# graz-dev/llms-on-kubernetes

Hardware: AMD Instinct MI355X
Metric: output tok/s through gateway (p50 TTFT reported) (higher is better)
Workload: dtype bf16

## Files before the change

csrc/kernels/prefill_gemm_packed.hip:

```cpp
#include "hipserve/common.h"
#include "hipserve/kernels.h"

namespace hipserve {

constexpr int PW_T = 256;

constexpr int PW_GM = 8;
HS_DEVICE void pw_tile(int L, int tiles_m, int tiles_n, int& tm, int& tn) {
  const int grp = L / (PW_GM * tiles_n), first = grp * PW_GM;
  const int gsz = min(PW_GM, tiles_m - first);
  const int r = L - first * tiles_n;
  tm = first + r % gsz;
  tn = r / gsz;
}

HS_DEVICE void pw_barrier() {
  asm volatile("s_waitcnt lgkmcnt(0)" ::: "memory");
  __builtin_amdgcn_s_barrier();
  asm volatile("" ::: "memory");
}

HS_DEVICE void pw_mfma(f32x4& acc, const u32x4& w, const u32x4& x) {
  asm volatile("v_mfma_f32_16x16x32_bf16 %0, %1, %2, %0" : "+a"(acc) : "v"(w), "v"(x));
}

struct PwTile {
  __amdgpu_buffer_rsrc_t w, x;
  int m0, t;
  int xo[8];
};

template <int WM, bool kGroup, bool kGather = false>
HS_DEVICE PwTile pw_make(int L, int tiles_m, int tiles_n, int wn, const unsigned short* X, long ldx,
                         const unsigned short* Wp, int M, int ntiles, int KS, const PwGroup& grp) {
  constexpr int WN = 4 / WM, BM = 128 * WM;
  int tm, tn;
  pw_tile(L, tiles_m, tiles_n, tm, tn);
  PwTile T;
  T.m0 = tm * BM;
  T.t = tn * WN + wn;
  const int tl = min(T.t, ntiles - 1);
  if constexpr (kGroup) Wp += (long)__builtin_amdgcn_readfirstlane(grp.tile_expert[tm]) * grp.estride;
  T.w = __builtin_amdgcn_make_buffer_rsrc((void*)(Wp + (long)tl * KS * 32768), 0, KS * 65536, 0x00020000);
  if constexpr (kGather) {
    const int bytes = (int)((long)grp.x_rows * ldx * 2);
    T.x = __builtin_amdgcn_make_buffer_rsrc((void*)X, 0, bytes, 0x00020000);
    const int tid = threadIdx.x;
#pragma unroll
    for (int p = 0; p < BM / 32; ++p) {
      const int row = T.m0 + p * 32 + (tid >> 3);
      const int s = row < M ? grp.gather_slots[row] : -1;
      T.xo[p] = (s >= 0 ? (s / grp.gather_k) * (int)ldx * 2 : bytes) + (tid & 7) * 16;
    }
  } else {
    T.x = __builtin_amdgcn_make_buffer_rsrc((void*)(X + (long)T.m0 * ldx), 0,
                                            (int)((long)min(BM, M - T.m0) * ldx * 2), 0x00020000);
  }
  return T;
}

template <int WM, int EPI, bool kGroup, int RW, bool LDLY = false, bool kGather = false>
__global__ __launch_bounds__(PW_T) __attribute__((amdgpu_waves_per_eu(1, 1))) void pgw_kernel(
    const unsigned short* __restrict__ X, long ldx, const unsigned short* __restrict__ Wp,
    unsigned short* __restrict__ C, long ldc, int M, int N, int K, int tiles_m, int tiles_n,
    const unsigned short* __restrict__ bias, PwGroup grp) {
  constexpr int WN = 4 / WM, BM = 128 * WM, STAGE = BM * 128, XP = BM / 32;
  __shared__ __attribute__((aligned(1024))) unsigned char lds[2 * STAGE];
  const int tid = threadIdx.x, lane = tid & 63;
  const int wave = __builtin_amdgcn_readfirstlane(tid >> 6);
  const int wm = wave / WN, wn = wave - (wave / WN) * WN;
  const int ntiles = (N + 127) >> 7;
  const int KS = K >> 8, nq = K >> 5, nst = K >> 6;
  if constexpr (kGroup) tiles_m = min(tiles_m, __builtin_amdgcn_readfirstlane(*grp.num_tiles));
  const int total = tiles_m * tiles_n, G = gridDim.x;
  const int r = xcd_remap(blockIdx.x, G);
  if (r >= total) return;

  PwTile cur = pw_make<WM, kGroup, kGather>(r, tiles_m, tiles_n, wn, X, ldx, Wp, M, ntiles, KS, grp);
  PwTile nxt = r + G < total ? pw_make<WM, kGroup, kGather>(r + G, tiles_m, tiles_n, wn, X, ldx, Wp, M, ntiles, KS, grp) : cur;

  const int wvo = lane * 16;
  auto wload = [&](int q, int rg) -> u32x4 {
    const bool n = q >= nq;
    q = n ? q - nq : q;
    return __builtin_amdgcn_raw_buffer_load_b128(n ? nxt.w : cur.w, wvo, (q >> 3) * 65536 + rg * 8192 + (q & 7) * 1024,
                                                 0);
  };
  int xvo[XP];
#pragma unroll
  for (int p = 0; p < XP; ++p) xvo[p] = (p * 32 + (tid >> 3)) * (int)ldx * 2 + (tid & 7) * 16;
  const int xdo = (tid >> 3) * 128 + (((tid & 7) ^ ((tid >> 4) & 7)) * 16);
  constexpr int XS = RW / 2;
  u32x4 xst[XS][XP];
  auto xload = [&](int st, u32x4 (&xs)[XP]) {
    const bool n = st >= nst;
    st = n ? st - nst : st;
#pragma unroll
    for (int p = 0; p < XP; ++p)
      xs[p] = __builtin_amdgcn_raw_buffer_load_b128(n ? nxt.x : cur.x, kGather ? (n ? nxt.xo[p] : cur.xo[p]) : xvo[p],
                                                    st * 128, 0);
  };
  auto xstore = [&](int buf, const u32x4 (&xs)[XP]) {
#pragma unroll
    for (int p = 0; p < XP; ++p) *reinterpret_cast<u32x4*>(lds + buf * STAGE + p * 4096 + xdo) = xs[p];
  };
  const int fr = lane & 15, fq = lane >> 4, sw = (fr >> 1) & 7;
  const int foff = (wm * 128 + fr) * 128;
  const int ch[2] = {(fq ^ sw) * 16, ((4 + fq) ^ sw) * 16};
  auto xfrag = [&](int buf, int h, int i) -> u32x4 {
    return *reinterpret_cast<const u32x4*>(lds + buf * STAGE + foff + i * 2048 + ch[h]);
  };

  f32x4 acc[8][8];
  u32x4 w[RW][8], xa[8], xb[8];
  int wvoj[RW];
#pragma unroll
  for (int j = 0; j < RW; ++j) wvoj[j] = wvo + j * 1024;

  xload(0, xst[0]);
  xstore(0, xst[0]);
#pragma unroll
  for (int s = 1; s <= XS; ++s) xload(s, xst[s % XS]);
#pragma unroll
  for (int j = 0; j < RW; ++j)
#pragma unroll
    for (int rg = 0; rg < 8; ++rg) w[j][rg] = wload(j, rg);
  pw_barrier();
#pragma unroll
  for (int i = 0; i < 8; ++i) xa[i] = xfrag(0, 0, i);

  auto slot = [&](auto jc, int s0, const __amdgpu_buffer_rsrc_t& wrs, int wk) {
    constexpr int J = decltype(jc)::value, H = J & 1;
    const int s = s0 + J / 2, buf = s & 1;
    constexpr int XI = (J / 2 + 1) % XS;
#pragma unroll
    for (int rg = 0; rg < 8; ++rg) {
#pragma unroll
      for (int i = 0; i < 8; ++i) pw_mfma(acc[rg][i], w[J][rg], H ? xb[i] : xa[i]);
      if constexpr (LDLY) {
        if (rg > 0) w[J][rg - 1] = __builtin_amdgcn_raw_buffer_load_b128(wrs, wvoj[J], wk + (rg - 1) * 8192, 0);
        if (rg == 7) w[J][7] = __builtin_amdgcn_raw_buffer_load_b128(wrs, wvoj[J], wk + 7 * 8192, 0);
      } else {
        w[J][rg] = __builtin_amdgcn_raw_buffer_load_b128(wrs, wvoj[J], wk + rg * 8192, 0);
      }
      if constexpr (H == 0) {
        xb[rg] = xfrag(buf, 1, rg);
        if (rg == 2) xstore(buf ^ 1, xst[XI]);
        if (rg == 3) xload(s + 1 + XS, xst[XI]);
      } else {
        xa[rg] = xfrag(buf ^ 1, 0, rg);
      }
      __builtin_amdgcn_sched_barrier(0);
    }
    if constexpr (H == 0) pw_barrier();
  };
  using I0 = std::integral_constant<int, 0>;
  using I1 = std::integral_constant<int, 1>;
  using I2 = std::integral_constant<int, 2>;
  using I3 = std::integral_constant<int, 3>;

  for (int L = r;;) {
#pragma unroll
    for (int rg = 0; rg < 8; ++rg)
#pragma unroll
      for (int i = 0; i < 8; ++i) acc[rg][i] = f32x4{0.f, 0.f, 0.f, 0.f};
    for (int q0 = 0; q0 < nq; q0 += RW) {
      const int s0 = q0 >> 1;
      const bool wn = q0 + RW >= nq;
      const int wq = wn ? q0 + RW - nq : q0 + RW;
      const __amdgpu_buffer_rsrc_t wrs = wn ? nxt.w : cur.w;
      const int wk = (wq >> 3) * 65536 + (wq & 7) * 1024;
      slot(I0(), s0, wrs, wk);
      slot(I1(), s0, wrs, wk);
      if constexpr (RW == 4) {
        slot(I2(), s0, wrs, wk);
        slot(I3(), s0, wrs, wk);
      }
    }

    asm volatile("s_nop 7\n\ts_nop 7\n\ts_nop 7\n\ts_nop 7" ::: "memory");
    const int t = cur.t, mb = cur.m0 + wm * 128 + fr;
    if (t < ntiles) {
      if constexpr (EPI == PW_EPI_GLU || EPI == PW_EPI_GEGLU) {
        const int I = N >> 1;
#pragma unroll
        for (int i = 0; i < 8; ++i) {
          const int m = mb + 16 * i;
          if (m >= M) continue;
#pragma unroll
          for (int rg = 0; rg < 4; ++rg) {
            const int c = t * 64 + rg * 16 + 4 * fq;
            unsigned short o[4];
#pragma unroll
            for (int j = 0; j < 4; ++j) {
              const unsigned short g = f32_to_bf16(acc[rg][i][j]), u = f32_to_bf16(acc[rg + 4][i][j]);
              o[j] = EPI == PW_EPI_GEGLU ? gelu_mul1(g, u) : silu_mul1(g, u);
            }
            if (c < I)
              *reinterpret_cast<uint2*>(C + (long)m * ldc + c) =
                  uint2{(unsigned)o[0] | ((unsigned)o[1] << 16), (unsigned)o[2] | ((unsigned)o[3] << 16)};
          }
        }
      } else {
#pragma unroll
        for (int rg = 0; rg < 8; ++rg) {
          const int n = t * 128 + rg * 16 + 4 * fq;
          if (n >= N) continue;
          float bv[4] = {0.f, 0.f, 0.f, 0.f};
          if (bias != nullptr)
#pragma unroll
            for (int j = 0; j < 4; ++j) bv[j] = n + j < N ? bf16_to_f32(bias[n + j]) : 0.f;
#pragma unroll
          for (int i = 0; i < 8; ++i) {
            const int m = mb + 16 * i;
            if (m >= M) continue;
            uint2* dst = reinterpret_cast<uint2*>(C + (long)m * ldc + n);
            float o[4];
            if constexpr (EPI == PW_EPI_ADD) {
              const uint2 rv = *dst;
              const unsigned short rr[4] = {(unsigned short)(rv.x & 0xffff), (unsigned short)(rv.x >> 16),
                                            (unsigned short)(rv.y & 0xffff), (unsigned short)(rv.y >> 16)};
#pragma unroll
              for (int j = 0; j < 4; ++j) o[j] = bf16_to_f32(f32_to_bf16(acc[rg][i][j])) + bf16_to_f32(rr[j]);
            } else {
#pragma unroll
              for (int j = 0; j < 4; ++j) o[j] = acc[rg][i][j] + bv[j];
            }
            *dst = uint2{pack_bf16x2(o[0], o[1]), pack_bf16x2(o[2], o[3])};
          }
        }
      }
    }
    L += G;
    if (L >= total) break;
    cur = nxt;
    if (L + G < total) nxt = pw_make<WM, kGroup, kGather>(L + G, tiles_m, tiles_n, wn, X, ldx, Wp, M, ntiles, KS, grp);
  }
}

bool launch_prefill_gemm_packed(int epi, void* C, long ldc, const void* X, long ldx, const void* Wp, int M, int N,
                                int K, const void* bias, int wm, int grid_req, hipStream_t s, const PwGroup* group,
                                int rw) {
  const PwGroup grp = group != nullptr ? *group : PwGroup{nullptr, nullptr, 0};
  const bool grouped = group != nullptr;
  const bool gather = grouped && grp.gather_slots != nullptr;
  if (grouped && (bias != nullptr || epi == PW_EPI_ADD)) return false;
  if (gather && (grp.gather_k < 1 || (long)grp.x_rows * ldx * 2 >= (1L << 31) - 4096)) return false;
  if (M < 1 || N < 1 || K < 256 || K % 256 || (wm != 1 && wm != 2) || (rw != 2 && rw != 4 && rw != 5)) return false;
  const bool glu = epi == PW_EPI_GLU || epi == PW_EPI_GEGLU;
  if (glu && (N % 128 || bias != nullptr)) return false;
  if (epi == PW_EPI_ADD && bias != nullptr) return false;
  if ((long)(K / 256) * 65536 >= (1L << 31) || (long)128 * wm * ldx * 2 >= (1L << 31)) return false;
  const int BM = 128 * wm, WN = 4 / wm;
  const int tiles_m = (M + BM - 1) / BM, tiles_n = ((N + 127) / 128 + WN - 1) / WN;
  static int ncu = 0;
  if (ncu == 0) {
    int dev = 0;
    (void)hipGetDevice(&dev);
    if (hipDeviceGetAttribute(&ncu, hipDeviceAttributeMultiprocessorCount, dev) != hipSuccess || ncu < 1) ncu = 256;
  }
  const int total = tiles_m * tiles_n;
  const dim3 grid(min(total, grid_req > 0 ? grid_req : ncu));
  auto* x = static_cast<const unsigned short*>(X);
  auto* w = static_cast<const unsigned short*>(Wp);
  auto* c = static_cast<unsigned short*>(C);
  auto* b = static_cast<const unsigned short*>(bias);
#define PW_LAUNCH1(WM_, E_, RW_)                                                                               \
  do {                                                                                                         \
    if (gather)                                                                                                \
      pgw_kernel<WM_, E_, true, 4, false, true><<<grid, PW_T, 0, s>>>(x, ldx, w, c, ldc, M, N, K, tiles_m, tiles_n, b, grp); \
    else if (grouped)                                                                                          \
      pgw_kernel<WM_, E_, true, RW_><<<grid, PW_T, 0, s>>>(x, ldx, w, c, ldc, M, N, K, tiles_m, tiles_n, b, grp);  \
    else                                                                                                       \
      pgw_kernel<WM_, E_, false, RW_><<<grid, PW_T, 0, s>>>(x, ldx, w, c, ldc, M, N, K, tiles_m, tiles_n, b, grp); \
  } while (0)
#define PW_LAUNCH(WM_, E_)                                                                                   \
  do {                                                                                                       \
    if (rw == 4)                                                                                             \
      PW_LAUNCH1(WM_, E_, 4);                                                                                \
    else if (rw == 2)                                                                                        \
      PW_LAUNCH1(WM_, E_, 2);                                                                                \
    else if (grouped)                                                                                        \
      pgw_kernel<WM_, E_, true, 4, true><<<grid, PW_T, 0, s>>>(x, ldx, w, c, ldc, M, N, K, tiles_m, tiles_n, b, grp);  \
    else                                                                                                     \
      pgw_kernel<WM_, E_, false, 4, true><<<grid, PW_T, 0, s>>>(x, ldx, w, c, ldc, M, N, K, tiles_m, tiles_n, b, grp); \
  } while (0)
#define PW_EPIS(WM_)                                          \
  switch (epi) {                                              \
    case PW_EPI_STORE: PW_LAUNCH(WM_, PW_EPI_STORE); return true; \
    case PW_EPI_ADD: PW_LAUNCH(WM_, PW_EPI_ADD); return true;     \
    case PW_EPI_GLU: PW_LAUNCH(WM_, PW_EPI_GLU); return true;     \
    case PW_EPI_GEGLU: PW_LAUNCH(WM_, PW_EPI_GEGLU); return true; \
    default: return false;                                    \
  }
  if (wm == 1) {
    PW_EPIS(1)
  }
  PW_EPIS(2)
#undef PW_EPIS
#undef PW_LAUNCH
#undef PW_LAUNCH1
}

}
```

csrc/torch_bindings.cpp:

```cpp
#include <torch/library.h>
#include <ATen/ATen.h>
#include <ATen/hip/impl/HIPGuardImplMasqueradingAsCUDA.h>
#include <ATen/hip/impl/HIPStreamMasqueradingAsCUDA.h>

#include "hipserve/kernels.h"

namespace {

hipStream_t cur_stream() {
  return c10::hip::getCurrentHIPStreamMasqueradingAsCUDA().stream();
}

#define CHECK_DEV(x) TORCH_CHECK((x).is_cuda(), #x " must be a GPU tensor")
#define CHECK_BF16(x) TORCH_CHECK((x).scalar_type() == at::kBFloat16, #x " must be bf16")
#define CHECK_ROWMAJOR(x) TORCH_CHECK((x).stride(-1) == 1, #x " must have unit inner stride")
#define CHECK_CONTIG(x) TORCH_CHECK((x).is_contiguous(), #x " must be contiguous")

static void e4m3_out_args(const c10::optional<at::Tensor>& out8, const c10::optional<at::Tensor>& xs8,
                          const at::Tensor& out, void** o8, float** x8, const char* who);

void rmsnorm(at::Tensor& out, const at::Tensor& x, const at::Tensor& weight, double eps,
             const c10::optional<at::Tensor>& out8, const c10::optional<at::Tensor>& xs8) {
  CHECK_DEV(x); CHECK_BF16(x); CHECK_BF16(out); CHECK_ROWMAJOR(x); CHECK_ROWMAJOR(out);
  TORCH_CHECK(x.dim() == 2 && out.dim() == 2, "rmsnorm expects 2-D [rows, hidden]");
// ... 612 lines not shown
  TORCH_CHECK(logits.dim() == 2 && (logits.scalar_type() == at::kBFloat16 || logits.scalar_type() == at::kFloat));
  const int rows = logits.size(0);
  TORCH_CHECK(nreq.scalar_type() == at::kInt && nreq.numel() >= rows);
  TORCH_CHECK(out_ids.scalar_type() == at::kInt && out_lp.scalar_type() == at::kFloat && out_ids.dim() == 2 &&
              out_ids.sizes() == out_lp.sizes() && out_ids.size(0) >= rows && out_ids.is_contiguous() &&
              out_lp.is_contiguous() && out_ids.size(1) <= 64);
  c10::hip::HIPGuardMasqueradingAsCUDA g(logits.device());
  hipserve::launch_top_logprobs(logits.data_ptr(), logits.scalar_type() == at::kBFloat16, logits.stride(0), rows,
                                logits.size(1), nreq.data_ptr<int>(), out_ids.data_ptr<int>(),
                                out_lp.data_ptr<float>(), out_ids.size(1), cur_stream());
}

bool car_error(int64_t state) { return hipserve::car_error(reinterpret_cast<void*>(state)); }

void car_destroy(int64_t state) { hipserve::car_destroy(reinterpret_cast<void*>(state)); }

void fill_uniform(at::Tensor& out, int64_t row0, int64_t col0, int64_t gcols, int64_t key, double scale) {
  CHECK_DEV(out); CHECK_BF16(out);
  TORCH_CHECK(out.dim() == 2 && out.stride(1) == 1, "fill_uniform: 2-D row-major view");
  c10::hip::HIPGuardMasqueradingAsCUDA g(out.device());
  hipserve::launch_fill_uniform(out.data_ptr(), out.stride(0), out.size(0), out.size(1), row0, col0, gcols,
                                (unsigned int)(key & 0xffffffffu), (float)scale, cur_stream());
}

void stage_copy(const std::vector<at::Tensor>& dst, const std::vector<at::Tensor>& src, int64_t device) {
  TORCH_CHECK(dst.size() == src.size() && dst.size() <= (size_t)hipserve::kMaxStageCopies,
              "stage_copy: matching lists of at most 8 tensors");
  hipserve::StageCopyArgs a{};
  a.n = (int)dst.size();
  auto addr = [](const at::Tensor& t, bool& host) -> void* {
    TORCH_CHECK(t.is_contiguous(), "stage_copy: tensors must be contiguous");
    if (t.is_cuda()) { host = false; return t.data_ptr(); }
    TORCH_CHECK(t.is_pinned(), "stage_copy: host tensors must be pinned");
    host = true;
    void* d = nullptr;
    TORCH_CHECK(hipHostGetDevicePointer(&d, t.data_ptr(), 0) == hipSuccess && d,
                "stage_copy: pinned tensor has no device mapping");
    return d;
  };
  for (int i = 0; i < a.n; ++i) {
    const size_t nb = dst[i].nbytes();
    TORCH_CHECK(nb == src[i].nbytes() && nb % 4 == 0, "stage_copy: pair ", i, " byte sizes differ or not 4-aligned");
    bool hd = false, hs = false;
    a.dst[i] = addr(dst[i], hd);
    a.src[i] = addr(src[i], hs);
    a.words[i] = (long)(nb / 4);
    a.host_mask |= (hs ? 1u : 0u) << (2 * i);
    a.host_mask |= (hd ? 1u : 0u) << (2 * i + 1);
  }
  c10::hip::HIPGuardMasqueradingAsCUDA g((c10::DeviceIndex)device);
  hipserve::launch_stage_copy(a, cur_stream());
}

void decode_gemm(at::Tensor& out, const at::Tensor& x, const at::Tensor& w, at::Tensor& ws, int64_t rt,
                 int64_t splits) {
  CHECK_DEV(x); CHECK_BF16(x); CHECK_BF16(w); CHECK_BF16(out); CHECK_ROWMAJOR(x); CHECK_ROWMAJOR(out);
  CHECK_CONTIG(w);
  const int M = x.size(0), K = x.size(1), N = w.size(0);
  TORCH_CHECK(w.size(1) == K && out.size(0) == M && out.size(1) == N, "decode_gemm: shape mismatch");
  TORCH_CHECK(M >= 1 && M <= 64, "decode_gemm: 1 <= M <= 64");
  TORCH_CHECK(splits >= 1 && K % (256 * splits) == 0, "decode_gemm: K must be a multiple of 256*splits");
  TORCH_CHECK(N % 4 == 0 && out.stride(0) % 4 == 0 && x.stride(0) % 8 == 0, "decode_gemm: alignment");
  if (splits > 1) {
    TORCH_CHECK(ws.scalar_type() == at::kFloat && ws.is_contiguous() && ws.numel() >= splits * M * N && N % 8 == 0,
                "decode_gemm: fp32 workspace of S*M*N (N % 8 == 0) required for split-K");
  }
  c10::hip::HIPGuardMasqueradingAsCUDA g(x.device());
  TORCH_CHECK(hipserve::launch_decode_gemm(out.data_ptr(), out.stride(0),
                                           splits > 1 ? ws.data_ptr<float>() : nullptr, x.data_ptr(), x.stride(0),
                                           w.data_ptr(), M, N, K, rt, splits, false, 0, cur_stream()),
              "decode_gemm: unsupported (rt, K/splits): rt in {1,2}, K/splits = 256*{1,2,4,7,8,12,16,21}");
}

void decode_gemm_packed(at::Tensor& out, const at::Tensor& x, const at::Tensor& wp, at::Tensor& ws, int64_t N,
                        int64_t rt, int64_t splits) {
  CHECK_DEV(x); CHECK_BF16(x); CHECK_BF16(wp); CHECK_BF16(out); CHECK_ROWMAJOR(x); CHECK_ROWMAJOR(out);
  CHECK_CONTIG(wp);
  const int M = x.size(0), K = x.size(1);
  TORCH_CHECK(K % 256 == 0 && wp.numel() == (N + 127) / 128 * 128 * K, "decode_gemm_packed: packed size mismatch");
  TORCH_CHECK(out.size(0) == M && out.size(1) == N, "decode_gemm_packed: out shape");
  TORCH_CHECK(M >= 1 && M <= 64, "decode_gemm_packed: 1 <= M <= 64");
  TORCH_CHECK(splits >= 1 && K % (256 * splits) == 0, "decode_gemm_packed: K must be a multiple of 256*splits");
  TORCH_CHECK(N % 4 == 0 && out.stride(0) % 4 == 0 && x.stride(0) % 8 == 0, "decode_gemm_packed: alignment");
  if (splits > 1) {
    TORCH_CHECK(ws.scalar_type() == at::kFloat && ws.is_contiguous() && ws.numel() >= splits * M * N && N % 8 == 0,
                "decode_gemm_packed: fp32 workspace of S*M*N (N % 8 == 0) required for split-K");
  }
  c10::hip::HIPGuardMasqueradingAsCUDA g(x.device());
  TORCH_CHECK(hipserve::launch_decode_gemm(out.data_ptr(), out.stride(0),
                                           splits > 1 ? ws.data_ptr<float>() : nullptr, x.data_ptr(), x.stride(0),
                                           wp.data_ptr(), M, N, K, rt, splits, true, 0, cur_stream()),
              "decode_gemm_packed: unsupported (rt, K/splits)");
}

void decode_gemm_partial(at::Tensor& ws, const at::Tensor& x, const at::Tensor& w, int64_t N, int64_t rt,
                         int64_t splits, bool packed) {
  CHECK_DEV(x); CHECK_BF16(x); CHECK_BF16(w); CHECK_ROWMAJOR(x); CHECK_CONTIG(w);
  const int M = x.size(0), K = x.size(1);
  if (packed) {
    TORCH_CHECK(w.numel() == (N + 127) / 128 * 128 * K, "decode_gemm_partial: packed size mismatch");
  } else {
    TORCH_CHECK(w.dim() == 2 && w.size(0) == N && w.size(1) == K, "decode_gemm_partial: w [N, K]");
  }
  TORCH_CHECK(M >= 1 && M <= 64 && K % (256 * splits) == 0 && N % 8 == 0 && x.stride(0) % 8 == 0,
              "decode_gemm_partial: shape / alignment");
  TORCH_CHECK(ws.scalar_type() == at::kFloat && ws.is_contiguous() && ws.numel() >= splits * M * N,
              "decode_gemm_partial: ws must hold S*M*N fp32");
  c10::hip::HIPGuardMasqueradingAsCUDA g(x.device());
  TORCH_CHECK(hipserve::launch_decode_gemm(nullptr, N, ws.data_ptr<float>(), x.data_ptr(), x.stride(0), w.data_ptr(),
                                           M, N, K, rt, splits, packed, hipserve::DG_PARTIAL, cur_stream()),
              "decode_gemm_partial: unsupported (rt, K/splits)");
}

void decode_gemm_glu(at::Tensor& act, const at::Tensor& x, const at::Tensor& wp, at::Tensor& ws, int64_t N,
                     int64_t rt, int64_t splits) {
  CHECK_DEV(x); CHECK_BF16(x); CHECK_BF16(wp); CHECK_BF16(act); CHECK_ROWMAJOR(x); CHECK_ROWMAJOR(act);
  CHECK_CONTIG(wp);
  const int M = x.size(0), K = x.size(1);
  TORCH_CHECK(N % 128 == 0 && wp.numel() == N * K && K % (256 * splits) == 0, "decode_gemm_glu: shapes");
  TORCH_CHECK(act.size(0) == M && act.size(1) == N / 2 && act.stride(0) % 8 == 0, "decode_gemm_glu: act [M, N/2]");
  TORCH_CHECK(M >= 1 && M <= 64 && x.stride(0) % 8 == 0, "decode_gemm_glu: 1 <= M <= 64");
  if (splits > 1) {
    TORCH_CHECK(ws.scalar_type() == at::kFloat && ws.is_contiguous() && ws.numel() >= splits * M * N,
                "decode_gemm_glu: ws must hold S*M*N fp32");
  }
  c10::hip::HIPGuardMasqueradingAsCUDA g(x.device());
  TORCH_CHECK(hipserve::launch_decode_gemm(act.data_ptr(), act.stride(0), splits > 1 ? ws.data_ptr<float>() : nullptr,
                                           x.data_ptr(), x.stride(0), wp.data_ptr(), M, N, K, rt, splits, true,
                                           hipserve::DG_GLU, cur_stream()),
              "decode_gemm_glu: unsupported (rt, K/splits)");
}



void prefill_gemm_packed(at::Tensor& out, const at::Tensor& x, const at::Tensor& wp, int64_t N, int64_t epi,
                         const c10::optional<at::Tensor>& bias, int64_t wm, int64_t grid, int64_t rw) {
  CHECK_DEV(x); CHECK_BF16(x); CHECK_BF16(wp); CHECK_BF16(out); CHECK_ROWMAJOR(x); CHECK_ROWMAJOR(out);
  TORCH_CHECK(wp.is_contiguous(), "prefill_gemm_packed: packed weight must be contiguous");
  const int M = x.size(0), K = x.size(1);
  TORCH_CHECK(K % 256 == 0 && wp.numel() == (N + 127) / 128 * 128 * K, "prefill_gemm_packed: wp = pack(w[N, K % 256])");
  TORCH_CHECK(x.stride(0) % 8 == 0 && out.stride(0) % 4 == 0, "prefill_gemm_packed: alignment");
  const bool glu = epi == 2 || epi == 3;
  TORCH_CHECK(out.size(0) == M && out.size(1) == (glu ? N / 2 : N), "prefill_gemm_packed: out shape");
  const void* bp = nullptr;
  if (bias.has_value()) {
    CHECK_BF16((*bias));
    TORCH_CHECK(bias->numel() == N && bias->is_contiguous(), "prefill_gemm_packed: bias [N]");
    bp = bias->data_ptr();
  }
  c10::hip::HIPGuardMasqueradingAsCUDA g(x.device());
  TORCH_CHECK(hipserve::launch_prefill_gemm_packed((int)epi, out.data_ptr(), out.stride(0), x.data_ptr(), x.stride(0),
                                                   wp.data_ptr(), M, (int)N, K, bp, (int)wm, (int)grid, cur_stream(),
                                                   nullptr, (int)rw),
              "prefill_gemm_packed: unsupported (glu needs N % 128, bias only with epi 0, 32-bit offsets)");
}

void prefill_gemm_packed_grouped(at::Tensor& out, const at::Tensor& x, const at::Tensor& wp, int64_t N, int64_t epi,
                                 const at::Tensor& tile_expert, const at::Tensor& num_tiles, int64_t wm, int64_t rw,
                                 const c10::optional<at::Tensor>& gather_slots, int64_t gather_k) {
  CHECK_DEV(x); CHECK_BF16(x); CHECK_BF16(wp); CHECK_BF16(out); CHECK_ROWMAJOR(x); CHECK_ROWMAJOR(out);
  TORCH_CHECK(wp.dim() == 2 && wp.is_contiguous(), "prefill_gemm_packed_grouped: wp [E, packed]");
  const bool gather = gather_slots.has_value() && gather_slots->numel() > 0;
  if (gather)
    TORCH_CHECK(gather_slots->scalar_type() == at::kInt && gather_slots->is_contiguous() &&
                    gather_slots->numel() == out.size(0) && gather_k >= 1 && x.stride(0) % 8 == 0,
                "prefill_gemm_packed_grouped: gather_slots [slot rows] int32, gather_k >= 1");
  const int M = gather ? out.size(0) : x.size(0), K = x.size(1);
  TORCH_CHECK(K % 256 == 0 && wp.size(1) == (N + 127) / 128 * 128 * K, "prefill_gemm_packed_grouped: wp per expert");
  TORCH_CHECK(M % (128 * wm) == 0 && tile_expert.numel() >= M / (128 * wm), "prefill_gemm_packed_grouped: tiles");
  TORCH_CHECK(tile_expert.scalar_type() == at::kInt && num_tiles.scalar_type() == at::kInt, "int32 tile tables");
  const bool glu = epi == 2 || epi == 3;
  TORCH_CHECK(epi == 0 || glu, "prefill_gemm_packed_grouped: store or glu epilogue");
  TORCH_CHECK(out.size(0) == M && out.size(1) == (glu ? N / 2 : N), "prefill_gemm_packed_grouped: out shape");
  c10::hip::HIPGuardMasqueradingAsCUDA g(x.device());
  hipserve::PwGroup grp{tile_expert.data_ptr<int>(), num_tiles.data_ptr<int>(), (long)wp.size(1)};
  if (gather) {
    grp.gather_slots = gather_slots->data_ptr<int>();
    grp.gather_k = (int)gather_k;
    grp.x_rows = (int)x.size(0);
  }
  TORCH_CHECK(hipserve::launch_prefill_gemm_packed((int)epi, out.data_ptr(), out.stride(0), x.data_ptr(), x.stride(0),
                                                   wp.data_ptr(), M, (int)N, K, nullptr, (int)wm, 0, cur_stream(),
                                                   &grp, (int)rw),
              "prefill_gemm_packed_grouped: unsupported");
}

void prefill_gemm_f8(at::Tensor& out, const at::Tensor& xq, const at::Tensor& xs, const std::vector<at::Tensor>& q,
                     const std::vector<at::Tensor>& rs, int64_t epi) {
  CHECK_DEV(xq); CHECK_CONTIG(xq); CHECK_CONTIG(xs); CHECK_BF16(out); CHECK_ROWMAJOR(out);
  TORCH_CHECK(xq.scalar_type() == at::kByte && xs.scalar_type() == at::kFloat, "prefill_gemm_f8: xq uint8, xs fp32");
  const int M = xq.size(0), K = xq.size(1);
  TORCH_CHECK(xs.numel() == M && K % 256 == 0 && out.stride(0) % 4 == 0, "prefill_gemm_f8: shapes");
  TORCH_CHECK(!q.empty() && q.size() <= (size_t)hipserve::kPgF8Parts && rs.size() == q.size(), "prefill_gemm_f8: parts");
  hipserve::PgF8 W{};
  W.n = (int)q.size();
  W.xs = xs.data_ptr<float>();
  int rows = 0;
  for (size_t i = 0; i < q.size(); ++i) {
    CHECK_CONTIG(q[i]); CHECK_CONTIG(rs[i]);
    const int n = rs[i].numel();
    TORCH_CHECK(q[i].scalar_type() == at::kByte && rs[i].scalar_type() == at::kFloat && q[i].numel() == (long)n * K,
                "prefill_gemm_f8: part ", i, " must be tiled FP8 [N/16, K/256, 4096] with rs [N]");
    W.p[i] = hipserve::PgF8Part{q[i].data_ptr<uint8_t>(), rs[i].data_ptr<float>(), n, rows / 256};
    rows += n;
  }
  const bool glu = epi == 2 || epi == 3;
  TORCH_CHECK(out.size(0) == M && out.size(1) == (glu ? rows / 2 : rows), "prefill_gemm_f8: out shape");
  c10::hip::HIPGuardMasqueradingAsCUDA g(xq.device());
  TORCH_CHECK(hipserve::launch_prefill_gemm_f8((int)epi, out.data_ptr(), out.stride(0), xq.data_ptr(), K, W, M, rows, K,
                                               cur_stream()),
              "prefill_gemm_f8: unsupported part shapes (rows % 256; GLU: two equal parts, rows % 128)");
}

void fp8_decode_gemm(at::Tensor& ws, const at::Tensor& xq, const at::Tensor& xs, const std::vector<at::Tensor>& q,
                     const std::vector<at::Tensor>& rs, int64_t splits) {
  CHECK_DEV(xq); CHECK_CONTIG(xq); CHECK_CONTIG(xs); CHECK_CONTIG(ws);
  TORCH_CHECK(xq.scalar_type() == at::kByte && xs.scalar_type() == at::kFloat && ws.scalar_type() == at::kFloat,
              "fp8_decode_gemm: xq uint8, xs / ws fp32");
  const int M = xq.size(0), K = xq.size(1);
  TORCH_CHECK(xs.numel() == M && K % 256 == 0, "fp8_decode_gemm: shapes");
  TORCH_CHECK(!q.empty() && q.size() <= (size_t)hipserve::kPgF8Parts && rs.size() == q.size(), "fp8_decode_gemm: parts");
  hipserve::PgF8 W{};
  W.n = (int)q.size();
  W.xs = xs.data_ptr<float>();
  int rows = 0;
  for (size_t i = 0; i < q.size(); ++i) {
    CHECK_CONTIG(q[i]); CHECK_CONTIG(rs[i]);
    const int n = rs[i].numel();
    TORCH_CHECK(q[i].scalar_type() == at::kByte && rs[i].scalar_type() == at::kFloat && q[i].numel() == (long)n * K,
                "fp8_decode_gemm: part ", i, " must be tiled FP8 [N/16, K/256, 4096] with rs [N]");
    W.p[i] = hipserve::PgF8Part{q[i].data_ptr<uint8_t>(), rs[i].data_ptr<float>(), n, 0};
    rows += n;
  }
  TORCH_CHECK(ws.numel() >= splits * (long)M * rows, "fp8_decode_gemm: ws too small");
  c10::hip::HIPGuardMasqueradingAsCUDA g(xq.device());
  TORCH_CHECK(hipserve::launch_fp8_decode_gemm(ws.data_ptr<float>(), xq.data_ptr(), W, M, rows, K, (int)splits,
                                               cur_stream()),
              "fp8_decode_gemm: unsupported (M <= 256, part rows % 16, (K / 256) / splits in the kernel's step set)");
}

void glu_quant(const c10::optional<at::Tensor>& out, at::Tensor& q8, at::Tensor& xs, const at::Tensor& x, bool gelu) {
  CHECK_DEV(x); CHECK_BF16(x); CHECK_ROWMAJOR(x); CHECK_CONTIG(q8); CHECK_CONTIG(xs);
  const long rows = x.size(0);
  const int inter = x.size(1) / 2;
  TORCH_CHECK(q8.scalar_type() == at::kByte && q8.size(0) == rows && q8.size(1) == inter &&
                  xs.scalar_type() == at::kFloat && xs.numel() == rows && x.stride(0) % 8 == 0,
              "glu_quant: q8 uint8 [rows, I], xs fp32 [rows]");
  void* o = nullptr;
  if (out.has_value() && out->defined()) {
    TORCH_CHECK(out->scalar_type() == at::kBFloat16 && out->is_contiguous() && out->size(0) == rows &&
                out->size(1) == inter, "glu_quant: out bf16 [rows, I]");
    o = out->data_ptr();
  }
  c10::hip::HIPGuardMasqueradingAsCUDA g(x.device());
  TORCH_CHECK(hipserve::launch_glu_quant(gelu, o, q8.data_ptr(), xs.data_ptr<float>(), x.data_ptr(), rows, inter,
                                         x.stride(0), cur_stream()),
              "glu_quant: I % 8 == 0 and I <= 32768");
}

void act_quant_fp8(at::Tensor& xq, at::Tensor& xs, const at::Tensor& x) {
  CHECK_DEV(x); CHECK_BF16(x); CHECK_ROWMAJOR(x); CHECK_CONTIG(xq); CHECK_CONTIG(xs);
  const int M = x.size(0), K = x.size(1);
  TORCH_CHECK(xq.scalar_type() == at::kByte && xq.size(0) == M && xq.size(1) == K && xs.scalar_type() == at::kFloat &&
                  xs.numel() == M && K % 8 == 0 && x.stride(0) % 8 == 0,
              "act_quant_fp8: xq uint8 [M, K], xs fp32 [M], K % 8 == 0");
  c10::hip::HIPGuardMasqueradingAsCUDA g(x.device());
  hipserve::launch_act_quant_fp8(xq.data_ptr(), xs.data_ptr<float>(), x.data_ptr(), x.stride(0), M, K, cur_stream());
}


static const void* opt_ptr(const c10::optional<at::Tensor>& t) { return t.has_value() ? t->data_ptr() : nullptr; }

static void e4m3_out_args(const c10::optional<at::Tensor>& out8, const c10::optional<at::Tensor>& xs8,
                          const at::Tensor& out, void** o8, float** x8, const char* who) {
  *o8 = nullptr;
  *x8 = nullptr;
  if (out8.has_value() && out8->defined()) {
    TORCH_CHECK(xs8.has_value() && xs8->defined(), who, ": out8 needs xs8");
    TORCH_CHECK(out8->scalar_type() == at::kByte && out8->sizes() == out.sizes() && out8->is_contiguous() &&
                    xs8->scalar_type() == at::kFloat && xs8->numel() == out.size(0) && xs8->is_contiguous(),
                who, ": out8 uint8 like out, xs8 fp32 [M]");
    *o8 = out8->data_ptr();
    *x8 = xs8->data_ptr<float>();
  }
}

void splitk_add_rmsnorm(at::Tensor& out, at::Tensor& residual, const at::Tensor& ws, int64_t splits,
                        const at::Tensor& weight, double eps, const c10::optional<at::Tensor>& out16,
                        const c10::optional<at::Tensor>& out8, const c10::optional<at::Tensor>& xs8) {
  CHECK_DEV(ws); CHECK_BF16(out); CHECK_BF16(residual); CHECK_CONTIG(out); CHECK_CONTIG(residual);
  TORCH_CHECK(ws.scalar_type() == at::kFloat && ws.is_contiguous());
  const int M = residual.size(0), N = residual.size(1);
  TORCH_CHECK(out.sizes() == residual.sizes() && ws.numel() >= splits * M * N && N % 8 == 0 && N <= 16384);
  TORCH_CHECK(weight.numel() == N && weight.is_contiguous() &&
              (weight.scalar_type() == at::kBFloat16 || weight.scalar_type() == at::kFloat));
  c10::hip::HIPGuardMasqueradingAsCUDA g(ws.device());
  void* o16 = nullptr;
  if (out16.has_value() && out16->defined()) {
    TORCH_CHECK(out16->scalar_type() == at::kHalf && out16->sizes() == out.sizes() && out16->is_contiguous(),
                "splitk_add_rmsnorm: out16 f16 like out");
    o16 = out16->data_ptr();
  }
  void* o8;
  float* x8;
  e4m3_out_args(out8, xs8, out, &o8, &x8, "splitk_add_rmsnorm");
  hipserve::launch_splitk_add_rmsnorm(out.data_ptr(), residual.data_ptr(), ws.data_ptr<float>(), splits,
                                      weight.data_ptr(), weight.scalar_type() == at::kFloat, M, N, (float)eps,
// ... 404 lines not shown
```

Baseline: 7690.

## Widen GEMM epilogue stores, reschedule LDS fragment loads, force persistent grid for shapes

Rewrites the prefill GEMM epilogue to use buffer resources and permlane16_swap, so each lane writes 128-bit stores of two adjacent 16-column fragments instead of 64-bit stores. The residual-add path now reads with 128-bit buffer loads. The main loop issues LDS fragment reads two per step in the first half of each slot and moves the global x store and load to later steps. A waitcnt is added before the first barrier. A table of specific (N, K) shapes forces a persistent grid of one block per CU. This adds new alignment restrictions and hardcodes model-specific shapes.

Measured after the change: 7677, median of 2. No clear change (-0.2%).

```diff
diff --git a/csrc/kernels/prefill_gemm_packed.hip b/csrc/kernels/prefill_gemm_packed.hip
--- a/csrc/kernels/prefill_gemm_packed.hip
+++ b/csrc/kernels/prefill_gemm_packed.hip
@@ -22,6 +22,12 @@
 
 HS_DEVICE void pw_mfma(f32x4& acc, const u32x4& w, const u32x4& x) {
   asm volatile("v_mfma_f32_16x16x32_bf16 %0, %1, %2, %0" : "+a"(acc) : "v"(w), "v"(x));
+}
+
+HS_DEVICE u32x4 pw_widen(uint2 a, uint2 b) {
+  const auto lo = __builtin_amdgcn_permlane16_swap(a.x, b.x, false, false);
+  const auto hi = __builtin_amdgcn_permlane16_swap(a.y, b.y, false, false);
+  return u32x4{lo[0], hi[0], lo[1], hi[1]};
 }
 
 struct PwTile {
@@ -125,6 +131,7 @@
   for (int j = 0; j < RW; ++j)
 #pragma unroll
     for (int rg = 0; rg < 8; ++rg) w[j][rg] = wload(j, rg);
+  __builtin_amdgcn_s_waitcnt(0x0f70);
   pw_barrier();
 #pragma unroll
   for (int i = 0; i < 8; ++i) xa[i] = xfrag(0, 0, i);
@@ -144,11 +151,15 @@
         w[J][rg] = __builtin_amdgcn_raw_buffer_load_b128(wrs, wvoj[J], wk + rg * 8192, 0);
       }
       if constexpr (H == 0) {
-        xb[rg] = xfrag(buf, 1, rg);
-        if (rg == 2) xstore(buf ^ 1, xst[XI]);
-        if (rg == 3) xload(s + 1 + XS, xst[XI]);
-      } else {
-        xa[rg] = xfrag(buf ^ 1, 0, rg);
+        if (rg < 4) {
+          xb[2 * rg] = xfrag(buf, 1, 2 * rg);
+          xb[2 * rg + 1] = xfrag(buf, 1, 2 * rg + 1);
+        }
+        if (rg == 4) xstore(buf ^ 1, xst[XI]);
+        if (rg == 5) xload(s + 1 + XS, xst[XI]);
+      } else if (rg < 4) {
+        xa[2 * rg] = xfrag(buf ^ 1, 0, 2 * rg);
+        xa[2 * rg + 1] = xfrag(buf ^ 1, 0, 2 * rg + 1);
       }
       __builtin_amdgcn_sched_barrier(0);
     }
@@ -178,56 +189,65 @@
       }
     }
 
-    asm volatile("s_nop 7\n\ts_nop 7\n\ts_nop 7\n\ts_nop 7" ::: "memory");
-    const int t = cur.t, mb = cur.m0 + wm * 128 + fr;
+    asm volatile("s_nop 7\n\ts_nop 7\n\ts_nop 7\n\ts_nop 7"
+                 : "+a"(acc[7][0]), "+a"(acc[7][1]), "+a"(acc[7][2]), "+a"(acc[7][3]), "+a"(acc[7][4]), "+a"(acc[7][5]),
+                   "+a"(acc[7][6]), "+a"(acc[7][7])
+                 :
+                 : "memory");
+    const int t = cur.t;
     if (t < ntiles) {
-      if constexpr (EPI == PW_EPI_GLU || EPI == PW_EPI_GEGLU) {
-        const int I = N >> 1;
-#pragma unroll
-        for (int i = 0; i < 8; ++i) {
-          const int m = mb + 16 * i;
-          if (m >= M) continue;
-#pragma unroll
-          for (int rg = 0; rg < 4; ++rg) {
-            const int c = t * 64 + rg * 16 + 4 * fq;
+      constexpr bool kGlu = EPI == PW_EPI_GLU || EPI == PW_EPI_GEGLU;
+      const int ncol = kGlu ? N >> 1 : N;
+      const __amdgpu_buffer_rsrc_t crs = __builtin_amdgcn_make_buffer_rsrc(
+          (void*)(C + (long)cur.m0 * ldc), 0, (int)((long)min(BM, M - cur.m0) * ldc * 2), 0x00020000);
+      const unsigned rowo = (unsigned)(wm * 128 + fr) * (unsigned)ldc * 2u, rstep = 32u * (unsigned)ldc;
+#pragma unroll
+      for (int rp = 0; rp < (kGlu ? 2 : 4); ++rp) {
+        const int n8 = t * (kGlu ? 64 : 128) + rp * 32 + 16 * (fq & 1) + 8 * (fq >> 1);
+        const unsigned vo = n8 < ncol ? rowo + 2u * (unsigned)n8 : 0x80000000u;
+        float bv[2][4] = {{0.f, 0.f, 0.f, 0.f}, {0.f, 0.f, 0.f, 0.f}};
+        if constexpr (EPI == PW_EPI_STORE)
+          if (bias != nullptr)
+#pragma unroll
+            for (int h = 0; h < 2; ++h) {
+              const int n = t * 128 + (2 * rp + h) * 16 + 4 * fq;
+#pragma unroll
+              for (int j = 0; j < 4; ++j) bv[h][j] = n + j < N ? bf16_to_f32(bias[n + j]) : 0.f;
+            }
+        auto packed = [&](int h, int i) -> uint2 {
+          if constexpr (kGlu) {
             unsigned short o[4];
 #pragma unroll
             for (int j = 0; j < 4; ++j) {
-              const unsigned short g = f32_to_bf16(acc[rg][i][j]), u = f32_to_bf16(acc[rg + 4][i][j]);
+              const unsigned short g = f32_to_bf16(acc[2 * rp + h][i][j]), u = f32_to_bf16(acc[2 * rp + h + 4][i][j]);
               o[j] = EPI == PW_EPI_GEGLU ? gelu_mul1(g, u) : silu_mul1(g, u);
             }
-            if (c < I)
-              *reinterpret_cast<uint2*>(C + (long)m * ldc + c) =
-                  uint2{(unsigned)o[0] | ((unsigned)o[1] << 16), (unsigned)o[2] | ((unsigned)o[3] << 16)};
+            return uint2{(unsigned)o[0] | ((unsigned)o[1] << 16), (unsigned)o[2] | ((unsigned)o[3] << 16)};
+          } else if constexpr (EPI == PW_EPI_ADD) {
+            const f32x4& a = acc[2 * rp + h][i];
+            return uint2{pack_bf16x2(a[0], a[1]), pack_bf16x2(a[2], a[3])};
+          } else {
+            const f32x4& a = acc[2 * rp + h][i];
+            return uint2{pack_bf16x2(a[0] + bv[h][0], a[1] + bv[h][1]), pack_bf16x2(a[2] + bv[h][2], a[3] + bv[h][3])};
           }
-        }
-      } else {
-#pragma unroll
-        for (int rg = 0; rg < 8; ++rg) {
-          const int n = t * 128 + rg * 16 + 4 * fq;
-          if (n >= N) continue;
-          float bv[4] = {0.f, 0.f, 0.f, 0.f};
-          if (bias != nullptr)
-#pragma unroll
-            for (int j = 0; j < 4; ++j) bv[j] = n + j < N ? bf16_to_f32(bias[n + j]) : 0.f;
-#pragma unroll
-          for (int i = 0; i < 8; ++i) {
-            const int m = mb + 16 * i;
-            if (m >= M) continue;
-            uint2* dst = reinterpret_cast<uint2*>(C + (long)m * ldc + n);
-            float o[4];
-            if constexpr (EPI == PW_EPI_ADD) {
-              const uint2 rv = *dst;
-              const unsigned short rr[4] = {(unsigned short)(rv.x & 0xffff), (unsigned short)(rv.x >> 16),
-                                            (unsigned short)(rv.y & 0xffff), (unsigned short)(rv.y >> 16)};
-#pragma unroll
-              for (int j = 0; j < 4; ++j) o[j] = bf16_to_f32(f32_to_bf16(acc[rg][i][j])) + bf16_to_f32(rr[j]);
-            } else {
-#pragma unroll
-              for (int j = 0; j < 4; ++j) o[j] = acc[rg][i][j] + bv[j];
-            }
-            *dst = uint2{pack_bf16x2(o[0], o[1]), pack_bf16x2(o[2], o[3])};
-          }
+        };
+#pragma unroll
+        for (int i0 = 0; i0 < 8; i0 += 4) {
+          u32x4 v[4], rv[4];
+          if constexpr (EPI == PW_EPI_ADD)
+#pragma unroll
+            for (int i = 0; i < 4; ++i) rv[i] = __builtin_amdgcn_raw_buffer_load_b128(crs, vo + (i0 + i) * rstep, 0, 0);
+#pragma unroll
+          for (int i = 0; i < 4; ++i) v[i] = pw_widen(packed(0, i0 + i), packed(1, i0 + i));
+          if constexpr (EPI == PW_EPI_ADD)
+#pragma unroll
+            for (int i = 0; i < 4; ++i)
+#pragma unroll
+              for (int d = 0; d < 4; ++d)
+                v[i][d] = pack_bf16x2(__uint_as_float(v[i][d] << 16) + __uint_as_float(rv[i][d] << 16),
+                                      __uint_as_float(v[i][d] & 0xffff0000u) + __uint_as_float(rv[i][d] & 0xffff0000u));
+#pragma unroll
+          for (int i = 0; i < 4; ++i) __builtin_amdgcn_raw_buffer_store_b128(v[i], crs, vo + (i0 + i) * rstep, 0, 0);
         }
       }
     }
@@ -251,6 +271,7 @@
   if (glu && (N % 128 || bias != nullptr)) return false;
   if (epi == PW_EPI_ADD && bias != nullptr) return false;
   if ((long)(K / 256) * 65536 >= (1L << 31) || (long)128 * wm * ldx * 2 >= (1L << 31)) return false;
+  if ((glu ? N / 2 : N) % 8 || ldc % 2 || ((unsigned long)C & 3) || (long)128 * wm * ldc * 2 >= (1L << 31)) return false;
   const int BM = 128 * wm, WN = 4 / wm;
   const int tiles_m = (M + BM - 1) / BM, tiles_n = ((N + 127) / 128 + WN - 1) / WN;
   static int ncu = 0;
@@ -260,6 +281,11 @@
     if (hipDeviceGetAttribute(&ncu, hipDeviceAttributeMultiprocessorCount, dev) != hipSuccess || ncu < 1) ncu = 256;
   }
   const int total = tiles_m * tiles_n;
+  static const int kPersistent[][2] = {{6144, 4096},  {4096, 4096}, {28672, 4096}, {4096, 14336},
+                                       {10240, 8192}, {8192, 8192}, {8192, 28672}};
+  if (!grouped && wm == 1 && rw == 4 && grid_req >= total && total >= 2 * ncu)
+    for (const auto& u : kPersistent)
+      if (u[0] == N && u[1] == K) grid_req = ncu;
   const dim3 grid(min(total, grid_req > 0 ? grid_req : ncu));
   auto* x = static_cast<const unsigned short*>(X);
   auto* w = static_cast<const unsigned short*>(Wp);
diff --git a/csrc/torch_bindings.cpp b/csrc/torch_bindings.cpp
--- a/csrc/torch_bindings.cpp
+++ b/csrc/torch_bindings.cpp
@@ -788,7 +788,7 @@
   TORCH_CHECK(hipserve::launch_prefill_gemm_packed((int)epi, out.data_ptr(), out.stride(0), x.data_ptr(), x.stride(0),
                                                    wp.data_ptr(), M, (int)N, K, bp, (int)wm, (int)grid, cur_stream(),
                                                    nullptr, (int)rw),
-              "prefill_gemm_packed: unsupported (glu needs N % 128, bias only with epi 0, 32-bit offsets)");
+              "prefill_gemm_packed: unsupported (out columns % 8, glu needs N % 128, bias only with epi 0, 32-bit offsets)");
 }
 
 void prefill_gemm_packed_grouped(at::Tensor& out, const at::Tensor& x, const at::Tensor& wp, int64_t N, int64_t epi,
```
